# Gui-Yom/turbo-metrics

Measured on AMD Instinct MI355X. Metric: ssimulacra2_frame_pairs_per_sec, higher is better.
Workload: dtype f32; 1 GPU; 1080p_nv12; width=1920, height=1080, input=nv12, full_sums=False, parallelism=frame-pair sharding x1, one RCCL reduce of scores

## Files before the change

### turbo-metrics_amd/csrc/tm_platform.h

```cpp
#pragma once

#ifdef TM_EMULATE
#include "hip_emul.h"
#include <stdint.h>

namespace tmdev {
struct tm_f2 { float x, y; };
static inline tm_f2 operator*(tm_f2 a, tm_f2 b) { return {a.x * b.x, a.y * b.y}; }
static inline tm_f2 operator-(tm_f2 a, tm_f2 b) { return {a.x - b.x, a.y - b.y}; }
static inline tm_f2 operator+(tm_f2 a, tm_f2 b) { return {a.x + b.x, a.y + b.y}; }
static inline tm_f2 operator-(tm_f2 a) { return {-a.x, -a.y}; }
static inline tm_f2 f2_fma(tm_f2 a, tm_f2 b, tm_f2 c) { return {fmaf(a.x, b.x, c.x), fmaf(a.y, b.y, c.y)}; }
static inline float tm_fract_pos(float s) { return s - floorf(s); }
}

#define TM_WAVE_ANY(c) true
#define TM_WAVE_ALL(c) (c)
#define TM_NO_IF_CONVERSION() ((void)0)
#define TM_WAVES_PER_SIMD(n)
#define TM_LDS_BARRIER() __syncthreads()
#define TM_GLOBAL_AS
#define TM_PIN_SGPR(v) ((void)0)
#define TM_KEEP_IN_VGPR(v) ((void)0)
#define TM_SETPRIO(n) ((void)0)
#define TM_SLEEP(n) ((void)0)
#define TM_EF_SPIN_PAUSE() ::tm_emul_yield()
#define TM_EF_LDS_FENCE() __atomic_thread_fence(__ATOMIC_SEQ_CST)

struct alignas(16) tm_f4 { float x, y, z, w; };
struct alignas(8) tm_g2 { float x, y; };
struct alignas(8) tm_u2 { unsigned x, y; };
static inline unsigned tm_mul24(unsigned a, unsigned b) { return a * b; }
static inline float tm_swap1(float v) { return tm_shfl_xor(v, 1); }
static inline void tm_pair_values(float v, bool odd, float &even_v, float &odd_v)
{
    const float other = tm_swap1(v);
    even_v = odd ? other : v;
    odd_v = odd ? v : other;
}
static inline float tm_div_inrange(float n, float d) { return n / d; }
static inline float tm_rcp_inrange(float d) { return 1.0f / d; }
static inline void tm_ll_store(unsigned long long *p, float v, unsigned tag) { *(volatile unsigned long long *)p = ((unsigned long long)tag << 32) | __float_as_uint(v); }
static inline unsigned long long tm_ll_load(const unsigned long long *p) { return *(const volatile unsigned long long *)p; }

#else
#include <hip/hip_runtime.h>
#include <stdint.h>

namespace tmdev {
typedef float tm_f2 __attribute__((ext_vector_type(2)));
__device__ __forceinline__ tm_f2 f2_fma(tm_f2 a, tm_f2 b, tm_f2 c) { return __builtin_elementwise_fma(a, b, c); }
__device__ __forceinline__ float tm_fract_pos(float s) { return __builtin_amdgcn_fractf(s); }
}

#define TM_WAVE_ANY(c) (__builtin_amdgcn_ballot_w64(c) != 0ull)
#define TM_WAVE_ALL(c) (__builtin_amdgcn_ballot_w64(c) == ~0ull)
#define TM_NO_IF_CONVERSION() asm volatile("; rare path")
#define TM_WAVES_PER_SIMD(n) __attribute__((amdgpu_waves_per_eu(n)))
#define TM_LDS_BARRIER() asm volatile("s_waitcnt lgkmcnt(0)\n\ts_barrier" ::: "memory")
#define TM_GLOBAL_AS __attribute__((address_space(1)))
#define TM_PIN_SGPR(v) asm("" : "+s"(v))
#define TM_KEEP_IN_VGPR(v) asm volatile("" : "+v"(v))
#define TM_SETPRIO(n) __builtin_amdgcn_s_setprio(n)
#define TM_SLEEP(n) __builtin_amdgcn_s_sleep(n)
#define TM_EF_SPIN_PAUSE() __builtin_amdgcn_s_sleep(1)
#define TM_EF_LDS_FENCE() __builtin_amdgcn_fence(__ATOMIC_SEQ_CST, "workgroup")

typedef float tm_f4 __attribute__((ext_vector_type(4)));
typedef float tm_g2 __attribute__((ext_vector_type(2)));
typedef unsigned tm_u2 __attribute__((ext_vector_type(2)));

__device__ __forceinline__ bool tm_wave_sum6(double (&a)[6])
{
#pragma unroll
    for (int off = 32; off > 0; off >>= 1) {
#pragma unroll
        for (int k = 0; k < 6; ++k) a[k] += __shfl_down(a[k], off, 64);
    }
    return (threadIdx.x & 63) == 0;
}
__device__ __forceinline__ float tm_shfl_xor(float v, int mask) { return __shfl_xor(v, mask, 64); }
__device__ __forceinline__ unsigned tm_shfl_xor_u32(unsigned v, int mask) { return (unsigned)__shfl_xor((int)v, mask, 64); }
__device__ __forceinline__ bool tm_wave_sum_u32x3(unsigned (&v)[3])
{
#pragma unroll
    for (int off = 32; off > 0; off >>= 1) {
#pragma unroll
        for (int k = 0; k < 3; ++k) v[k] += __shfl_down(v[k], off, 64);
    }
    return ((threadIdx.x + threadIdx.y * blockDim.x) & 63) == 0;
}

__device__ __forceinline__ unsigned tm_mul24(unsigned a, unsigned b) { return __umul24(a, b); }
__device__ __forceinline__ float tm_swap1(float v)
{
    return __uint_as_float((unsigned)__builtin_amdgcn_mov_dpp((int)__float_as_uint(v), 0xB1, 0xF, 0xF, true));
}
__device__ __forceinline__ void tm_pair_values(float v, bool, float &even_v, float &odd_v)
{
    even_v = __uint_as_float((unsigned)__builtin_amdgcn_mov_dpp((int)__float_as_uint(v), 0xA0, 0xF, 0xF, true));
    odd_v = __uint_as_float((unsigned)__builtin_amdgcn_mov_dpp((int)__float_as_uint(v), 0xF5, 0xF, 0xF, true));
}
__device__ __forceinline__ float tm_div_inrange(float n, float d)
{
    const float r0 = __builtin_amdgcn_rcpf(d);
    const float r1 = __builtin_fmaf(__builtin_fmaf(-d, r0, 1.0f), r0, r0);
    const float q0 = n * r1;
    const float q1 = __builtin_fmaf(__builtin_fmaf(-d, q0, n), r1, q0);
    return __builtin_fmaf(__builtin_fmaf(-d, q1, n), r1, q1);
}
__device__ __forceinline__ float tm_rcp_inrange(float d)
{
    const float r0 = __builtin_amdgcn_rcpf(d);
    const float r1 = __builtin_fmaf(__builtin_fmaf(-d, r0, 1.0f), r0, r0);
    const float q1 = __builtin_fmaf(__builtin_fmaf(-d, r1, 1.0f), r1, r1);
    return __builtin_fmaf(__builtin_fmaf(-d, q1, 1.0f), r1, q1);
}
__device__ __forceinline__ void tm_ll_store(unsigned long long *p, float v, unsigned tag)
{
    __hip_atomic_store(p, ((unsigned long long)tag << 32) | __float_as_uint(v), __ATOMIC_RELAXED, __HIP_MEMORY_SCOPE_AGENT);
}
__device__ __forceinline__ unsigned long long tm_ll_load(const unsigned long long *p) { return __hip_atomic_load(p, __ATOMIC_RELAXED, __HIP_MEMORY_SCOPE_AGENT); }

#endif
```

### turbo-metrics_amd/csrc/tm_ssim_kernels.h

```cpp
#pragma once
#include "tm_device_math.h"
#include "tm_geom.h"

#define TM_SSIM_SCALES 5
#define TM_SSIM_TAPS 11
#define TM_SSIM_STRIP 118
#define TM_SSIM_SEG 192

struct TmSsimGeom {
    int w[TM_SSIM_SCALES], h[TM_SSIM_SCALES];
    int pitch[TM_SSIM_SCALES];
    unsigned long long off[TM_SSIM_SCALES];
    unsigned long long qplane;
    unsigned long long pyr;
    int strips_x[TM_SSIM_SCALES], segs_y[TM_SSIM_SCALES], seg_rows[TM_SSIM_SCALES];
    int item_off[TM_SSIM_SCALES + 1];
    float g[TM_SSIM_TAPS];
};

static inline void tm_make_ssim_geom(TmSsimGeom *s, int w, int h, const float g[TM_SSIM_TAPS])
{
    unsigned long long off = 0;
    s->item_off[0] = 0;
    for (int i = 0; i < TM_SSIM_SCALES; ++i) {
        s->w[i] = w; s->h[i] = h;
        s->pitch[i] = tm_round_up(w > 0 ? w : 1, 64);
        s->off[i] = off;
        if (i > 0) off += (unsigned long long)(h > 0 ? h : 1) * s->pitch[i];
        const int ow = w - 10, oh = h - 10;
        s->strips_x[i] = ow > 0 ? (ow + TM_SSIM_STRIP - 1) / TM_SSIM_STRIP : 0;
        s->segs_y[i] = oh > 0 ? (oh + TM_SSIM_SEG - 1) / TM_SSIM_SEG : 0;
        s->seg_rows[i] = s->segs_y[i] > 0 ? (oh + s->segs_y[i] - 1) / s->segs_y[i] : 0;
        s->item_off[i + 1] = s->item_off[i] + s->strips_x[i] * s->segs_y[i];
        w /= 2; h /= 2;
    }
    s->qplane = (unsigned long long)s->h[0] * s->pitch[0];
    s->pyr = off;
    for (int k = 0; k < TM_SSIM_TAPS; ++k) s->g[k] = g[k];
}

namespace tmk {

__device__ __forceinline__ const unsigned short *ssim_plane_s(const TmSsimGeom &sg, const unsigned short *PYR, int img, int c, int s)
{
    return PYR + ((size_t)img * 3 + c) * sg.pyr + sg.off[s];
}

__global__ void __launch_bounds__(64) k_ssim_pyramid(TmSsimGeom sg, const unsigned char *__restrict__ Q, unsigned short *__restrict__ PYR)
{
    const int lane = threadIdx.x;
    const int img = blockIdx.z / 3, c = blockIdx.z % 3;
    const int x0 = blockIdx.x * 128 + 8 * (lane & 15), y0 = blockIdx.y * 32 + 8 * (lane >> 4);
    const bool live = x0 < sg.pitch[0];
    const unsigned char *q = Q + ((size_t)img * 3 + c) * sg.qplane + x0;
    unsigned short *base = PYR + ((size_t)img * 3 + c) * sg.pyr;
    const int h = sg.h[0];
    unsigned l1[4][2];
#pragma unroll
    for (int j = 0; j < 4; ++j) {
        unsigned hs[2][2];
#pragma unroll
        for (int i = 0; i < 2; ++i) {
            const int y = min(y0 + 2 * j + i, h - 1);
            const uint2 u = live ? *(const uint2 *)(q + (size_t)y * sg.pitch[0]) : make_uint2(0u, 0u);
            hs[i][0] = (u.x & 0x00FF00FFu) + ((u.x >> 8) & 0x00FF00FFu);
            hs[i][1] = (u.y & 0x00FF00FFu) + ((u.y >> 8) & 0x00FF00FFu);
        }
        l1[j][0] = hs[0][0] + hs[1][0];
        l1[j][1] = hs[0][1] + hs[1][1];
    }
    const int x1 = x0 >> 1, y1 = y0 >> 1, x2 = x0 >> 2, y2 = y0 >> 2, x3 = x0 >> 3, y3 = y0 >> 3;
    if (x1 < sg.w[1])
#pragma unroll
        for (int j = 0; j < 4; ++j)
            if (y1 + j < sg.h[1]) *(uint2 *)(base + sg.off[1] + (size_t)(y1 + j) * sg.pitch[1] + x1) = make_uint2(l1[j][0], l1[j][1]);
    unsigned l2[2];
#pragma unroll
    for (int j = 0; j < 2; ++j) {
        const unsigned a = l1[2 * j][0] + l1[2 * j + 1][0], b = l1[2 * j][1] + l1[2 * j + 1][1];
        l2[j] = ((a & 0xFFFFu) + (a >> 16)) | (((b & 0xFFFFu) + (b >> 16)) << 16);
    }
    if (x2 < sg.w[2])
#pragma unroll
        for (int j = 0; j < 2; ++j)
            if (y2 + j < sg.h[2]) *(unsigned *)(base + sg.off[2] + (size_t)(y2 + j) * sg.pitch[2] + x2) = l2[j];
    const unsigned t = l2[0] + l2[1];
    const unsigned l3 = (t & 0xFFFFu) + (t >> 16);
    if (x3 < sg.w[3] && y3 < sg.h[3]) base[sg.off[3] + (size_t)y3 * sg.pitch[3] + x3] = (unsigned short)l3;
    const unsigned l4 = (l3 + tm_shfl_xor_u32(l3, 1)) + (tm_shfl_xor_u32(l3, 16) + tm_shfl_xor_u32(l3, 17));
    if (!(lane & 1) && !(lane & 16) && (x0 >> 4) < sg.w[4] && (y0 >> 4) < sg.h[4])
        base[sg.off[4] + (size_t)(y0 >> 4) * sg.pitch[4] + (x0 >> 4)] = (unsigned short)l4;
}

__device__ __forceinline__ float ssim_div(float n, float d) { return tm_div_inrange(n, d); }

struct __attribute__((aligned(16))) TmSsimCol { tmdev::tm_f2 rd, sp; };

template <bool S0, bool NEED_L>
__device__ __forceinline__ void ssim_strip(TmSsimCol *__restrict__ bufE, TmSsimCol *__restrict__ bufO, const void *__restrict__ pr, const void *__restrict__ pd,
                                           int pitch, float inv, int w, int h, int x, int y_base, int y_end, const float (&gw)[TM_SSIM_TAPS],
                                           double (&acc)[2])
{
    using tmdev::tm_f2;
    using tmdev::f2_fma;
    using tmdev::f2_make;
    using tmdev::f2_splat;
    const int lane = threadIdx.x & 63;
    const bool in0 = x < w, in1 = x + 1 < w;
    auto load = [&](int y, unsigned &a, unsigned &b) {
        const int yc = y < h ? y : h - 1;
        const size_t ro = (size_t)yc * (size_t)pitch * (S0 ? 1 : 2);
        TM_GLOBAL_AS const char *ra = (TM_GLOBAL_AS const char *)tm_uniform_ptr((const char *)pr + ro);
        TM_GLOBAL_AS const char *rb = (TM_GLOBAL_AS const char *)tm_uniform_ptr((const char *)pd + ro);
        const unsigned xo = in0 ? (unsigned)x * (S0 ? 1u : 2u) : 0u;
        unsigned va, vb;
        if (S0) { va = *(TM_GLOBAL_AS const unsigned short *)(ra + xo); vb = *(TM_GLOBAL_AS const unsigned short *)(rb + xo); }
        else { va = *(TM_GLOBAL_AS const unsigned *)(ra + xo); vb = *(TM_GLOBAL_AS const unsigned *)(rb + xo); }
        a = va; b = vb;
        (void)y;
    };
    auto unpack = [&](unsigned raw, int y, float &v0, float &v1) {
        if (S0) { v0 = (float)(raw & 255u); v1 = (float)((raw >> 8) & 255u); }
        else { v0 = (float)(raw & 0xFFFFu) * inv; v1 = (float)(raw >> 16) * inv; }
        const bool ok = y < h;
        if (!(ok && in0)) v0 = 0.0f;
        if (!(ok && in1)) v1 = 0.0f;
    };
    constexpr int PF = 3, WS = 12;
    static_assert(WS % PF == 0 && WS > TM_SSIM_TAPS, "ring and window sizes");
    unsigned pa[PF], pb[PF];
#pragma unroll
    for (int k = 0; k < PF; ++k) load(y_base + k, pa[k], pb[k]);
    tm_f2 g2[TM_SSIM_TAPS];
#pragma unroll
    for (int k = 0; k < TM_SSIM_TAPS; ++k) g2[k] = f2_splat(gw[k]);
    tm_f2 w01[WS][2], w23[WS][2];
#pragma unroll
    for (int k = 0; k < WS; ++k) { w01[k][0] = w01[k][1] = w23[k][0] = w23[k][1] = f2_splat(0.0f); }
    const tm_f2 C1 = f2_splat(6.5025f), C2 = f2_splat(58.5225f), two = f2_splat(2.0f);
    double a_l[2] = {0.0, 0.0}, a_cs[2] = {0.0, 0.0};
    const int n_rows = (y_end - y_base) + 10;
    for (int t0 = 0; t0 < n_rows; t0 += WS) {
#pragma unroll
        for (int j = 0; j < WS; ++j) {
            const int t = t0 + j;
            {
                float r0, r1, d0, d1;
                unpack(pa[j % PF], y_base + t, r0, r1);
                unpack(pb[j % PF], y_base + t, d0, d1);
                load(y_base + t + PF, pa[j % PF], pb[j % PF]);
                TmSsimCol c[12];
                c[0].rd = f2_make(r0, d0); c[0].sp = f2_make(__builtin_fmaf(r0, r0, d0 * d0), r0 * d0);
                c[1].rd = f2_make(r1, d1); c[1].sp = f2_make(__builtin_fmaf(r1, r1, d1 * d1), r1 * d1);
                __builtin_amdgcn_wave_barrier();
                bufE[lane] = c[0]; bufO[lane] = c[1];
                __builtin_amdgcn_wave_barrier();
#pragma unroll
                for (int i = 1; i < 6; ++i) { c[2 * i] = bufE[lane + i]; c[2 * i + 1] = bufO[lane + i]; }
                tm_f2 a01[2] = {f2_splat(0.0f), f2_splat(0.0f)}, a23[2] = {f2_splat(0.0f), f2_splat(0.0f)};
#pragma unroll
                for (int i = 0; i < 12; ++i) {
                    if (i < 11) { a01[0] = f2_fma(g2[i], c[i].rd, a01[0]); a23[0] = f2_fma(g2[i], c[i].sp, a23[0]); }
                    if (i > 0) { a01[1] = f2_fma(g2[i - 1], c[i].rd, a01[1]); a23[1] = f2_fma(g2[i - 1], c[i].sp, a23[1]); }
                }
                w01[j][0] = a01[0]; w01[j][1] = a01[1]; w23[j][0] = a23[0]; w23[j][1] = a23[1];
                if (t >= 10 && t < n_rows) {
                    tm_f2 v01[2] = {f2_splat(0.0f), f2_splat(0.0f)}, v23[2] = {f2_splat(0.0f), f2_splat(0.0f)};
#pragma unroll
                    for (int k = 0; k < TM_SSIM_TAPS; ++k) {
                        const int q = (j + WS - 10 + k) % WS;
                        v01[0] = f2_fma(g2[k], w01[q][0], v01[0]); v01[1] = f2_fma(g2[k], w01[q][1], v01[1]);
                        v23[0] = f2_fma(g2[k], w23[q][0], v23[0]); v23[1] = f2_fma(g2[k], w23[q][1], v23[1]);
                    }
                    const tm_f2 mx = f2_make(v01[0].x, v01[1].x), my = f2_make(v01[0].y, v01[1].y);
                    const tm_f2 mxx = mx * mx, myy = my * my, mxy = mx * my, mm = mxx + myy;
                    const tm_f2 sv = f2_make(v23[0].x, v23[1].x) - mm, sxy = f2_make(v23[0].y, v23[1].y) - mxy;
                    const tm_f2 csn = f2_fma(two, sxy, C2), csd = sv + C2;
                    const float cs0 = ssim_div(csn.x, csd.x), cs1 = ssim_div(csn.y, csd.y);
                    a_cs[0] += (double)cs0; a_cs[1] += (double)cs1;
                    if (NEED_L) {
                        const tm_f2 ln = f2_fma(two, mxy, C1), ld = mm + C1;
                        const float l0 = ssim_div(ln.x, ld.x), l1 = ssim_div(ln.y, ld.y);
                        a_l[0] += (double)(l0 * cs0); a_l[1] += (double)(l1 * cs1);
                    }
                }
            }
        }
    }
    const bool ok0 = 2 * lane < TM_SSIM_STRIP && x < w - 10, ok1 = 2 * lane + 1 < TM_SSIM_STRIP && x + 1 < w - 10;
    acc[0] = (ok0 ? a_l[0] : 0.0) + (ok1 ? a_l[1] : 0.0);
    acc[1] = (ok0 ? a_cs[0] : 0.0) + (ok1 ? a_cs[1] : 0.0);
}

#ifndef TM_SSIM_WAVES
#define TM_SSIM_WAVES 3
#endif
__global__ void __launch_bounds__(64) TM_WAVES_PER_SIMD(TM_SSIM_WAVES) k_ssim_stream(TmSsimGeom sg, int nscales, unsigned need_l, const unsigned char *__restrict__ Q,
                                                                         const unsigned short *__restrict__ PYR, double *__restrict__ PART)
{
    __shared__ TmSsimCol bufE[72], bufO[72];
    const int lane = threadIdx.x;
    const int slot = blockIdx.x / 3, c = blockIdx.x % 3;
    int s = 0;
#pragma unroll
    for (int i = 1; i < TM_SSIM_SCALES; ++i)
        if (i < nscales && (int)blockIdx.y >= sg.item_off[i]) s = i;
    const int item = (int)blockIdx.y - sg.item_off[s];
    const int w = sg.w[s], h = sg.h[s];
    const int x_base = (item % sg.strips_x[s]) * TM_SSIM_STRIP, y_base = (item / sg.strips_x[s]) * sg.seg_rows[s];
    const int y_end = min(y_base + sg.seg_rows[s], h - 10);
    const int x = x_base + 2 * lane;
    if (lane < 8) {
        TmSsimCol z; z.rd = z.sp = tmdev::f2_splat(0.0f);
        bufE[64 + lane] = z; bufO[64 + lane] = z;
    }
    float gw[TM_SSIM_TAPS];
#pragma unroll
    for (int k = 0; k < TM_SSIM_TAPS; ++k) gw[k] = sg.g[k];
    double acc[2] = {0.0, 0.0};
    const bool nl = (need_l >> s) & 1u;
    if (s == 0) {
        const unsigned char *qr = Q + ((size_t)(slot * 2 + 0) * 3 + c) * sg.qplane, *qd = Q + ((size_t)(slot * 2 + 1) * 3 + c) * sg.qplane;
        if (nl) ssim_strip<true, true>(bufE, bufO, qr, qd, sg.pitch[0], 1.0f, w, h, x, y_base, y_end, gw, acc);
        else ssim_strip<true, false>(bufE, bufO, qr, qd, sg.pitch[0], 1.0f, w, h, x, y_base, y_end, gw, acc);
    } else {
        const unsigned short *fr = ssim_plane_s(sg, PYR, slot * 2 + 0, c, s), *fd = ssim_plane_s(sg, PYR, slot * 2 + 1, c, s);
        const float inv = 1.0f / (float)(1 << (2 * s));
        if (nl) ssim_strip<false, true>(bufE, bufO, fr, fd, sg.pitch[s], inv, w, h, x, y_base, y_end, gw, acc);
        else ssim_strip<false, false>(bufE, bufO, fr, fd, sg.pitch[s], inv, w, h, x, y_base, y_end, gw, acc);
    }
    double a6[6] = {acc[0], acc[1], 0, 0, 0, 0};
    if (tm_wave_sum6(a6)) {
        double *o = PART + (((size_t)slot * 3 + c) * sg.item_off[TM_SSIM_SCALES] + blockIdx.y) * 2;
        o[0] = a6[0]; o[1] = a6[1];
    }
}

__global__ void __launch_bounds__(64) k_ssim_finish(TmSsimGeom sg, int nscales, const double *__restrict__ PART, double *__restrict__ SUMS)
{
    const int slot = blockIdx.x, i = blockIdx.y;
    const int c = i / 10, s = (i % 10) / 2, which = i & 1;
    double a[6] = {0, 0, 0, 0, 0, 0};
    if (s < nscales)
        for (int t = sg.item_off[s] + (int)threadIdx.x; t < sg.item_off[s + 1]; t += 64)
            a[0] += PART[(((size_t)slot * 3 + c) * sg.item_off[TM_SSIM_SCALES] + t) * 2 + which];
    if (tm_wave_sum6(a)) SUMS[(size_t)slot * 30 + i] = a[0];
}

}
```

Measured before the change: 14510 frame-pairs/s.

## Fold pyramid scale into SSIM constants, vectorize divisions, drop per-row masking

Removes the per-sample multiply by the inverse scale factor in the SSIM strip kernel. SSIM is scale-invariant in its ratios, so it instead scales the C1/C2 constants by the squared factor. The two per-column divisions are replaced by a packed two-wide Newton-refined division, and the per-row validity masking of loaded pixels (y<h, x<w zeroing) is removed, with clamped loads used instead. The row offset is also computed in 32-bit. This cuts VALU work in the inner loop, but dropping the zero-masking changes the values seen at the edge columns and rows, and exactness depends on the unscaled sums staying within float precision.

```diff
diff --git a/turbo-metrics_amd/csrc/tm_platform.h b/turbo-metrics_amd/csrc/tm_platform.h
--- a/turbo-metrics_amd/csrc/tm_platform.h
+++ b/turbo-metrics_amd/csrc/tm_platform.h
@@ -39,6 +39,7 @@
     odd_v = odd ? v : other;
 }
 static inline float tm_div_inrange(float n, float d) { return n / d; }
+static inline tmdev::tm_f2 tm_div_inrange2(tmdev::tm_f2 n, tmdev::tm_f2 d) { return {n.x / d.x, n.y / d.y}; }
 static inline float tm_rcp_inrange(float d) { return 1.0f / d; }
 static inline void tm_ll_store(unsigned long long *p, float v, unsigned tag) { *(volatile unsigned long long *)p = ((unsigned long long)tag << 32) | __float_as_uint(v); }
 static inline unsigned long long tm_ll_load(const unsigned long long *p) { return *(const volatile unsigned long long *)p; }
@@ -109,6 +110,17 @@
     const float q1 = __builtin_fmaf(__builtin_fmaf(-d, q0, n), r1, q0);
     return __builtin_fmaf(__builtin_fmaf(-d, q1, n), r1, q1);
 }
+__device__ __forceinline__ tmdev::tm_f2 tm_div_inrange2(tmdev::tm_f2 n, tmdev::tm_f2 d)
+{
+    using tmdev::f2_fma;
+    tmdev::tm_f2 r0, one;
+    r0.x = __builtin_amdgcn_rcpf(d.x); r0.y = __builtin_amdgcn_rcpf(d.y);
+    one.x = one.y = 1.0f;
+    const tmdev::tm_f2 r1 = f2_fma(f2_fma(-d, r0, one), r0, r0);
+    const tmdev::tm_f2 q0 = n * r1;
+    const tmdev::tm_f2 q1 = f2_fma(f2_fma(-d, q0, n), r1, q0);
+    return f2_fma(f2_fma(-d, q1, n), r1, q1);
+}
 __device__ __forceinline__ float tm_rcp_inrange(float d)
 {
     const float r0 = __builtin_amdgcn_rcpf(d);
diff --git a/turbo-metrics_amd/csrc/tm_ssim_kernels.h b/turbo-metrics_amd/csrc/tm_ssim_kernels.h
--- a/turbo-metrics_amd/csrc/tm_ssim_kernels.h
+++ b/turbo-metrics_amd/csrc/tm_ssim_kernels.h
@@ -92,13 +92,11 @@
         base[sg.off[4] + (size_t)(y0 >> 4) * sg.pitch[4] + (x0 >> 4)] = (unsigned short)l4;
 }
 
-__device__ __forceinline__ float ssim_div(float n, float d) { return tm_div_inrange(n, d); }
-
-struct __attribute__((aligned(16))) TmSsimCol { tmdev::tm_f2 rd, sp; };
+struct __attribute__((aligned(16))) TmSsimCol { tmdev::tm_f2 rd, ps; };
 
 template <bool S0, bool NEED_L>
 __device__ __forceinline__ void ssim_strip(TmSsimCol *__restrict__ bufE, TmSsimCol *__restrict__ bufO, const void *__restrict__ pr, const void *__restrict__ pd,
-                                           int pitch, float inv, int w, int h, int x, int y_base, int y_end, const float (&gw)[TM_SSIM_TAPS],
+                                           int pitch, float cscale, int w, int h, int x, int y_base, int y_end, const float (&gw)[TM_SSIM_TAPS],
                                            double (&acc)[2])
 {
     using tmdev::tm_f2;
@@ -106,26 +104,24 @@
     using tmdev::f2_make;
     using tmdev::f2_splat;
     const int lane = threadIdx.x & 63;
-    const bool in0 = x < w, in1 = x + 1 < w;
+    unsigned xo = x < w ? (unsigned)x * (S0 ? 1u : 2u) : 0u;
     auto load = [&](int y, unsigned &a, unsigned &b) {
         const int yc = y < h ? y : h - 1;
-        const size_t ro = (size_t)yc * (size_t)pitch * (S0 ? 1 : 2);
+        const unsigned ro = (unsigned)yc * ((unsigned)pitch * (S0 ? 1u : 2u));
         TM_GLOBAL_AS const char *ra = (TM_GLOBAL_AS const char *)tm_uniform_ptr((const char *)pr + ro);
         TM_GLOBAL_AS const char *rb = (TM_GLOBAL_AS const char *)tm_uniform_ptr((const char *)pd + ro);
-        const unsigned xo = in0 ? (unsigned)x * (S0 ? 1u : 2u) : 0u;
+        TM_KEEP_IN_VGPR(xo);
         unsigned va, vb;
         if (S0) { va = *(TM_GLOBAL_AS const unsigned short *)(ra + xo); vb = *(TM_GLOBAL_AS const unsigned short *)(rb + xo); }
         else { va = *(TM_GLOBAL_AS const unsigned *)(ra + xo); vb = *(TM_GLOBAL_AS const unsigned *)(rb + xo); }
         a = va; b = vb;
-        (void)y;
     };
-    auto unpack = [&](unsigned raw, int y, float &v0, float &v1) {
+    auto unpack = [&](unsigned raw, float &v0, float &v1) {
         if (S0) { v0 = (float)(raw & 255u); v1 = (float)((raw >> 8) & 255u); }
-        else { v0 = (float)(raw & 0xFFFFu) * inv; v1 = (float)(raw >> 16) * inv; }
-        const bool ok = y < h;
-        if (!(ok && in0)) v0 = 0.0f;
-        if (!(ok && in1)) v1 = 0.0f;
+        else { v0 = (float)(raw & 0xFFFFu); v1 = (float)(raw >> 16); }
+        TM_KEEP_IN_VGPR(v0); TM_KEEP_IN_VGPR(v1);
     };
+    auto products = [&](float r, float d) { return f2_make(r * d, __builtin_fmaf(r, r, d * d)); };
     constexpr int PF = 3, WS = 12;
     static_assert(WS % PF == 0 && WS > TM_SSIM_TAPS, "ring and window sizes");
     unsigned pa[PF], pb[PF];
@@ -137,7 +133,7 @@
     tm_f2 w01[WS][2], w23[WS][2];
 #pragma unroll
     for (int k = 0; k < WS; ++k) { w01[k][0] = w01[k][1] = w23[k][0] = w23[k][1] = f2_splat(0.0f); }
-    const tm_f2 C1 = f2_splat(6.5025f), C2 = f2_splat(58.5225f), two = f2_splat(2.0f);
+    const float C1 = 6.5025f * cscale, C2 = 58.5225f * cscale;
     double a_l[2] = {0.0, 0.0}, a_cs[2] = {0.0, 0.0};
     const int n_rows = (y_end - y_base) + 10;
     for (int t0 = 0; t0 < n_rows; t0 += WS) {
@@ -146,12 +142,12 @@
             const int t = t0 + j;
             {
                 float r0, r1, d0, d1;
-                unpack(pa[j % PF], y_base + t, r0, r1);
-                unpack(pb[j % PF], y_base + t, d0, d1);
+                unpack(pa[j % PF], r0, r1);
+                unpack(pb[j % PF], d0, d1);
                 load(y_base + t + PF, pa[j % PF], pb[j % PF]);
                 TmSsimCol c[12];
-                c[0].rd = f2_make(r0, d0); c[0].sp = f2_make(__builtin_fmaf(r0, r0, d0 * d0), r0 * d0);
-                c[1].rd = f2_make(r1, d1); c[1].sp = f2_make(__builtin_fmaf(r1, r1, d1 * d1), r1 * d1);
+                c[0].rd = f2_make(r0, d0); c[0].ps = products(r0, d0);
+                c[1].rd = f2_make(r1, d1); c[1].ps = products(r1, d1);
                 __builtin_amdgcn_wave_barrier();
                 bufE[lane] = c[0]; bufO[lane] = c[1];
                 __builtin_amdgcn_wave_barrier();
@@ -160,11 +156,11 @@
                 tm_f2 a01[2] = {f2_splat(0.0f), f2_splat(0.0f)}, a23[2] = {f2_splat(0.0f), f2_splat(0.0f)};
 #pragma unroll
                 for (int i = 0; i < 12; ++i) {
-                    if (i < 11) { a01[0] = f2_fma(g2[i], c[i].rd, a01[0]); a23[0] = f2_fma(g2[i], c[i].sp, a23[0]); }
-                    if (i > 0) { a01[1] = f2_fma(g2[i - 1], c[i].rd, a01[1]); a23[1] = f2_fma(g2[i - 1], c[i].sp, a23[1]); }
+                    if (i < 11) { a01[0] = f2_fma(g2[i], c[i].rd, a01[0]); a23[0] = f2_fma(g2[i], c[i].ps, a23[0]); }
+                    if (i > 0) { a01[1] = f2_fma(g2[i - 1], c[i].rd, a01[1]); a23[1] = f2_fma(g2[i - 1], c[i].ps, a23[1]); }
                 }
                 w01[j][0] = a01[0]; w01[j][1] = a01[1]; w23[j][0] = a23[0]; w23[j][1] = a23[1];
-                if (t >= 10 && t < n_rows) {
+                if ((unsigned)(t - 10) < (unsigned)(n_rows - 10)) {
                     tm_f2 v01[2] = {f2_splat(0.0f), f2_splat(0.0f)}, v23[2] = {f2_splat(0.0f), f2_splat(0.0f)};
 #pragma unroll
                     for (int k = 0; k < TM_SSIM_TAPS; ++k) {
@@ -174,14 +170,14 @@
                     }
                     const tm_f2 mx = f2_make(v01[0].x, v01[1].x), my = f2_make(v01[0].y, v01[1].y);
                     const tm_f2 mxx = mx * mx, myy = my * my, mxy = mx * my, mm = mxx + myy;
-                    const tm_f2 sv = f2_make(v23[0].x, v23[1].x) - mm, sxy = f2_make(v23[0].y, v23[1].y) - mxy;
-                    const tm_f2 csn = f2_fma(two, sxy, C2), csd = sv + C2;
-                    const float cs0 = ssim_div(csn.x, csd.x), cs1 = ssim_div(csn.y, csd.y);
-                    a_cs[0] += (double)cs0; a_cs[1] += (double)cs1;
+                    const tm_f2 sxy = f2_make(v23[0].x, v23[1].x) - mxy, sv = f2_make(v23[0].y, v23[1].y) - mm;
+                    const tm_f2 csn = f2_fma(f2_splat(2.0f), sxy, f2_splat(C2)), csd = sv + f2_splat(C2);
+                    const tm_f2 cs = tm_div_inrange2(csn, csd);
+                    a_cs[0] += (double)cs.x; a_cs[1] += (double)cs.y;
                     if (NEED_L) {
-                        const tm_f2 ln = f2_fma(two, mxy, C1), ld = mm + C1;
-                        const float l0 = ssim_div(ln.x, ld.x), l1 = ssim_div(ln.y, ld.y);
-                        a_l[0] += (double)(l0 * cs0); a_l[1] += (double)(l1 * cs1);
+                        const tm_f2 ln = f2_fma(f2_splat(2.0f), mxy, f2_splat(C1)), ld = mm + f2_splat(C1);
+                        const tm_f2 lcs = tm_div_inrange2(ln, ld) * cs;
+                        a_l[0] += (double)lcs.x; a_l[1] += (double)lcs.y;
                     }
                 }
             }
@@ -211,7 +207,7 @@
     const int y_end = min(y_base + sg.seg_rows[s], h - 10);
     const int x = x_base + 2 * lane;
     if (lane < 8) {
-        TmSsimCol z; z.rd = z.sp = tmdev::f2_splat(0.0f);
+        TmSsimCol z; z.rd = z.ps = tmdev::f2_splat(0.0f);
         bufE[64 + lane] = z; bufO[64 + lane] = z;
     }
     float gw[TM_SSIM_TAPS];
@@ -225,9 +221,9 @@
         else ssim_strip<true, false>(bufE, bufO, qr, qd, sg.pitch[0], 1.0f, w, h, x, y_base, y_end, gw, acc);
     } else {
         const unsigned short *fr = ssim_plane_s(sg, PYR, slot * 2 + 0, c, s), *fd = ssim_plane_s(sg, PYR, slot * 2 + 1, c, s);
-        const float inv = 1.0f / (float)(1 << (2 * s));
-        if (nl) ssim_strip<false, true>(bufE, bufO, fr, fd, sg.pitch[s], inv, w, h, x, y_base, y_end, gw, acc);
-        else ssim_strip<false, false>(bufE, bufO, fr, fd, sg.pitch[s], inv, w, h, x, y_base, y_end, gw, acc);
+        const float cscale = (float)(1 << (4 * s));
+        if (nl) ssim_strip<false, true>(bufE, bufO, fr, fd, sg.pitch[s], cscale, w, h, x, y_base, y_end, gw, acc);
+        else ssim_strip<false, false>(bufE, bufO, fr, fd, sg.pitch[s], cscale, w, h, x, y_base, y_end, gw, acc);
     }
     double a6[6] = {acc[0], acc[1], 0, 0, 0, 0};
     if (tm_wave_sum6(a6)) {
```

After: 14490 frame-pairs/s. No clear change (-0.1%).
